# ndmarco/BayesFMMM

Measured on AMD Instinct MI355X. Metric: Gibbs iterations/sec (whole node) at n_funct=4096, K=3, P=30, higher is better.
Workload: dtype f64; 1 GPU; BFMMM_warm_start sweep, n_funct=4096, n_i=100, K=3, P=30, M=6, fp64, one independent chain per GPU (1 chain(s): a chain does not shard, replicas only); chains=1, chains_per_gpu=1

## Files before the change

### bayesfmmm_amd/_lib.py

```python
import ctypes as C
import os

_HERE = os.path.dirname(os.path.abspath(__file__))
LIB_PATH = os.environ.get("BFMMM_LIB_PATH", os.path.join(_HERE, "libbfmmm_hip.so"))

c_double_p = C.POINTER(C.c_double)
c_int64_p = C.POINTER(C.c_int64)


class BfmmmConfig(C.Structure):
    _fields_ = [("model", C.c_int32), ("n_funct", C.c_int32), ("K", C.c_int32), ("n_eigen", C.c_int32),
                ("basis_degree", C.c_int32), ("n_internal_knots", C.c_int32), ("P", C.c_int32),
                ("tot_mcmc_iters", C.c_int32), ("c", C.c_double * 8), ("b", C.c_double), ("nu_1", C.c_double),
                ("alpha1l", C.c_double), ("alpha2l", C.c_double), ("beta1l", C.c_double), ("beta2l", C.c_double),
                ("a_Z_PM", C.c_double), ("a_pi_PM", C.c_double), ("var_alpha3", C.c_double),
                ("var_epsilon1", C.c_double), ("var_epsilon2", C.c_double), ("alpha_nu", C.c_double),
                ("beta_nu", C.c_double), ("alpha_eta", C.c_double), ("beta_eta", C.c_double),
                ("alpha_0", C.c_double), ("beta_0", C.c_double)]


SYMBOLS = {
    "bfmmm_config_defaults": (None, [C.POINTER(BfmmmConfig)]),
    "bfmmm_create": (C.c_int, [C.POINTER(BfmmmConfig), C.c_int, c_double_p, c_double_p, c_int64_p, c_double_p,
                               c_double_p, C.POINTER(C.c_void_p)]),
    "bfmmm_destroy": (None, [C.c_void_p]),
    "bfmmm_create_batch": (C.c_int, [C.POINTER(BfmmmConfig), C.c_int, c_double_p, c_double_p, c_int64_p, c_double_p,
                                     c_double_p, C.c_int, C.POINTER(C.c_void_p)]),
    "bfmmm_create_from_basis_batch": (C.c_int, [C.POINTER(BfmmmConfig), C.c_int, c_double_p, c_double_p, c_int64_p, C.c_int,
                                                C.c_int, c_double_p, C.c_int, C.c_int, C.POINTER(C.c_void_p)]),
    "bfmmm_select_chain": (C.c_int, [C.c_void_p, C.c_int]),
    "bfmmm_n_chains": (C.c_int, [C.c_void_p]),
    "bfmmm_set_chain_id_stride": (C.c_int, [C.c_void_p, C.c_uint32]),
    "bfmmm_gather_best": (C.c_int, [C.POINTER(C.c_void_p), C.c_int, c_double_p, C.POINTER(C.c_int32), C.POINTER(C.c_int)]),
    "bfmmm_set_covariates": (C.c_int, [C.c_void_p, c_double_p, C.c_int, C.c_int]),
    "bfmmm_get_basis": (C.c_int, [C.c_void_p, c_double_p, C.c_int64]),
    "bfmmm_set_state": (C.c_int, [C.c_void_p, C.c_char_p, c_double_p, C.c_int64]),
    "bfmmm_get_state": (C.c_int, [C.c_void_p, C.c_char_p, c_double_p, C.c_int64]),
    "bfmmm_init_state": (C.c_int, [C.c_void_p, C.c_int, C.c_uint64, C.c_uint32]),
    "bfmmm_run": (C.c_int, [C.c_void_p, C.c_uint32, C.c_int, C.c_int, C.c_uint64, C.c_uint32, C.c_int, C.c_double]),
    "bfmmm_prepare_run": (C.c_int, [C.c_void_p, C.c_uint32, C.c_int, C.c_int, C.c_uint64, C.c_uint32, C.c_int]),
    "bfmmm_set_slot_base": (C.c_int, [C.c_void_p, C.c_int]),
    "bfmmm_create_from_basis": (C.c_int, [C.POINTER(BfmmmConfig), C.c_int, c_double_p, c_double_p, c_int64_p, C.c_int, C.c_int,
                                          c_double_p, C.c_int, C.POINTER(C.c_void_p)]),
    "bfmmm_tempered_transition": (C.c_int, [C.c_void_p, C.c_uint32, C.c_int, C.c_int, C.c_double, C.c_uint64, C.c_uint32,
                                            c_double_p, C.POINTER(C.c_int)]),
    "bfmmm_get_chain": (C.c_int, [C.c_void_p, C.c_char_p, C.c_int, c_double_p, C.c_int64]),
    "bfmmm_chain_diagnostics": (C.c_int, [C.c_void_p, C.c_char_p, C.c_int, C.c_int, C.c_int64, c_double_p, c_double_p, c_double_p,
                                          c_double_p, c_double_p, c_double_p, c_double_p, C.c_int64]),
    "bfmmm_debug_get": (C.c_int, [C.c_void_p, C.c_char_p, c_double_p, C.c_int64, c_int64_p]),
    "bfmmm_set_profile": (C.c_int, [C.c_void_p, C.c_int]),
    "bfmmm_get_timing": (C.c_int, [C.c_void_p, C.c_char_p, C.POINTER(C.c_double), c_int64_p]),
    "bfmmm_set_exact_instances": (None, [C.c_int]),
    "bfmmm_last_error": (C.c_char_p, []),
}

_LIB = None


def load():
    global _LIB
    if _LIB is None:
        if not os.path.exists(LIB_PATH):
            raise RuntimeError(
                f"{LIB_PATH} is missing: build it with `python -c 'import __graft_entry__ as g; g.build()'` "
                "(hipcc --offload-arch=gfx950). bayesfmmm_amd has no CPU fallback.")
        lib = C.CDLL(LIB_PATH)
        for name, (res, args) in SYMBOLS.items():
            fn = getattr(lib, name)
            fn.restype = res
            fn.argtypes = args
        _LIB = lib
    return _LIB


class BfmmmError(RuntimeError):
    pass


def check(rc):
    if rc != 0:
        raise BfmmmError(load().bfmmm_last_error().decode())
```

### bayesfmmm_amd/csrc/bfmmm_capi.hip

```cpp
#include "../../include/bfmmm.h"
#include "model.hpp"
#include "rng.hpp"

#include <algorithm>
#include <cmath>
#include <cstdio>
#include <cstring>
#include <map>
#include <chrono>
#include <mutex>
#include <string>
#include <tuple>
#include <vector>

namespace bfmmm {
int launch_stats_functional(int degree, int n, int P, int LREC, const int64_t* off, const double* t, const double* y,
                            const double* knots, int n_knots, double* rec, int* ni, double* B_dense, int* err,
                            hipStream_t st);
void launch_stats_multivariate(int n, int P, int LREC, const double* Y, double* rec, int* ni, hipStream_t st);
void launch_stats_totals(int n, int LREC, int yy_off, const double* rec, const int* ni, double* out_yy,
                         long long* out_counts, hipStream_t st);
int launch_curve(const Ctx& c, int which, int do_update, hipStream_t st);
int curve_blocks(int n, int P);
void prepare_curve_kernels();
// ... 921 lines not shown
  c.seed = seed; c.chain = chain; c.mask = mask;
  Plan plan = make_plan(mask, MD);
  if (c.d.D > 0) { plan.z = true; plan.chi = true; plan.use_rss_part = 1; }
  c.defer_loglik = (c.d.D == 0) ? 1 : 0;
  c.ll_use_part = plan.use_rss_part;
  h->last_md = MD;
  int nsub = 1;
  if (!h->profile && h->nch >= 4) nsub = 2;
  if (const char* env_split = h->profile ? nullptr : getenv("BFMMM_BATCH_SPLIT"))
    nsub = std::max(1, std::min({atoi(env_split), (int)bfmmm_handle::MAX_SUB, h->nch / 2}));
  Sub subs[bfmmm_handle::MAX_SUB];
  h->sub_st[0] = h->st;
  for (int q = 0, q0 = 0; q < nsub; ++q) {
    const int cnt = h->nch / nsub + (q < h->nch % nsub ? 1 : 0);
    if (pg_route(h, c.d, plan.pg, cnt, h->profile ? bfmmm_handle::MAX_SUB : q, subs[q].r)) return 1;
    if (!h->sub_st[q]) HIPCHK(hipStreamCreateWithFlags(&h->sub_st[q], hipStreamNonBlocking));
    if (!h->sub_ev[q]) HIPCHK(hipEventCreateWithFlags(&h->sub_ev[q], hipEventDisableTiming));
    subs[q].c = chain_ctx(c, (unsigned)q0);
    subs[q].c.nch = cnt;
    subs[q].st = h->sub_st[q];
    q0 += cnt;
  }
  c.defer_hyper = (c.defer_loglik && plan.pg && plan.chi && h->nch == 1 && !subs[0].r.packed && subs[0].r.NKS >= 2) ? 1 : 0;
  subs[0].c.defer_hyper = c.defer_hyper;
  if (!prepare_only) {
    ensure_sweep_tables(h, c, mask);
    hipLaunchKernelGGL(k_run_begin, dim3(h->nch), dim3(64), 0, h->st, h->c, (uint32_t)first_iter, (uint32_t)h->slot_base, tt_step, beta,
                       h->state_dirty ? 1 : 0);
    h->state_dirty = false;
    for (int f = 0; f < FAM_COUNT; ++f) { h->fam_ms[f] = 0; h->fam_launches[f] = 0; }
  }
  if (h->profile) {
    if (prepare_only) return 0;
    HIPCHK(hipEventRecord(h->ev0, h->st));
    if (run_profiled(h, c, plan, subs[0].r, n_iters, tt_step)) return 1;
    return finish_run(h, c, plan, mask, first_iter, n_iters, false);
  }
  const bool fuse = plan.z && plan.z_update && plan.chi && c.d.D == 0 && n_iters >= 2 && tt_step == 0;
  const bool defer = !fuse && plan.z && plan.z_update && plan.factor && (mask & U_Z) && c.d.D == 0 && c.d.K <= 4 && c.d.BW <= 5 &&
                     n_iters >= 2 && tt_step == 0;
  const bool bodies = fuse || defer;
  const int body_kind = fuse ? GK_FUSED : GK_DEFERRED;
  const int nrep = bodies ? n_iters - 1 : n_iters;
  const bool whole = bodies && nsub == 1 && n_iters <= WHOLE_MAX && c.defer_loglik && h->status_dev != nullptr;
  std::vector<std::pair<int, int>> segs;
  const int kind = bodies ? body_kind : GK_FULL;
  if (whole) {
    segs.push_back({GK_WHOLE, n_iters});
  } else {
    for (int q = 0; q < nrep / GRAPH_UNROLL; ++q) segs.push_back({kind, GRAPH_UNROLL});
    if (nrep % GRAPH_UNROLL) segs.push_back({kind, nrep % GRAPH_UNROLL});
    if (bodies) segs.push_back({GK_CLOSING, 1});
  }
  const bfmmm_handle::GraphKey key{mask, MD, seed, chain, nsub, bfmmm::g_exact_instances ? 1 : 0};
  if (n_iters > 0 && !(h->g_valid && h->g_key == key)) { drop_graphs(h); h->g_key = key; h->g_valid = true; }
  std::vector<FreshGraph> fresh;
  std::vector<hipGraphExec_t> seq[bfmmm_handle::MAX_SUB];
  for (int s = 0; s < nsub; ++s)
    for (const auto& sg : segs) {
      hipGraphExec_t g = nullptr;
      if (cached_graph(h, s, sg.first, sg.second, subs[s].st, fresh, [&]() { queue_graph(h, c, subs[s], plan, sg.first, sg.second, body_kind); }, &g))
        return 1;
      seq[s].push_back(g);
    }
  if (prepare_only) return dry_launch(h, c, mask, subs, nsub, fresh, first_iter, tt_step, beta);
  HIPCHK(hipEventRecord(h->ev0, h->st));
  if (nsub > 1) HIPCHK(hipEventRecord(h->evA, h->st));
  for (int q = 1; q < nsub; ++q) HIPCHK(hipStreamWaitEvent(subs[q].st, h->evA, 0));
  for (int s = 0; s < nsub && n_iters > 0; ++s) {
    if (bodies && !whole) launch_curve(subs[s].c, 0, plan.z_update, subs[s].st);
    for (hipGraphExec_t g : seq[s]) HIPCHK(hipGraphLaunch(g, subs[s].st));
  }
  for (int q = 1; q < nsub; ++q) { HIPCHK(hipEventRecord(h->sub_ev[q], subs[q].st)); HIPCHK(hipStreamWaitEvent(h->st, h->sub_ev[q], 0)); }
  return finish_run(h, c, plan, mask, first_iter, n_iters, whole);
}

extern "C" int bfmmm_set_slot_base(bfmmm_handle* h, int base) {
  if (!h || base < 0) return fail("bfmmm_set_slot_base: bad arguments");
  h->slot_base = base;
  return 0;
}

extern "C" int bfmmm_run(bfmmm_handle* h, uint32_t mask, int first_iter, int n_iters, uint64_t seed, uint32_t chain,
                         int phi_chi_zero, double beta) {
  return run_impl(h, mask, first_iter, n_iters, seed, chain, phi_chi_zero, beta, 0);
}

extern "C" int bfmmm_prepare_run(bfmmm_handle* h, uint32_t mask, int first_iter, int n_iters, uint64_t seed, uint32_t chain,
                                 int phi_chi_zero) {
  return run_impl(h, mask, first_iter, n_iters, seed, chain, phi_chi_zero, 1.0, 0, true);
}

extern "C" int bfmmm_tempered_transition(bfmmm_handle* h, uint32_t mask, int iter, int N_t, double beta_N_t,
                                         uint64_t seed, uint32_t chain, double* logA_out, int* accepted_out) {
  if (!h) return fail("bfmmm_tempered_transition: null handle");
  if (N_t < 1 || iter < h->slot_base || iter - h->slot_base >= h->T) return fail("bfmmm_tempered_transition: bad arguments");
  if (h->nch != 1) return fail("bfmmm_tempered_transition: a tempered transition accepts or rejects one chain: not available on a chain batch");
  HIPCHK(hipSetDevice(h->device));
  const Ctx& c = h->c;
  const Dims& d = c.d;
  const size_t n_th = (size_t)d.K * (d.M + 1) * d.P, n_chi = (size_t)d.n * d.M, n_Z = (size_t)d.n * d.K,
               n_dl = (size_t)d.K * d.M, n_A = (size_t)d.K * 2, n_g = (size_t)d.K * d.P * d.M;
  const size_t Dc = (size_t)d.D;
  const size_t n_tx = (size_t)d.K * (d.M + 1) * Dc * d.P, n_te = (size_t)d.K * Dc, n_gx = (size_t)d.K * d.P * Dc * d.M,
               n_dx = (size_t)d.K * d.M * Dc, n_ax = (size_t)d.K * 2 * Dc;
  if (!h->tt_save) { if (dalloc(h, &h->tt_save, n_th + n_chi + n_Z + n_dl + n_A + n_g + n_tx + n_te + n_gx + n_dx + n_ax + 8)) return 1; }
  double* sv = h->tt_save;
// ... 151 lines not shown
  HIPCHK(hipMalloc(&d_ws, per_row * (size_t)chunk));
  double* d_x = d_ws;
  double* d_out = d_x + (size_t)chunk * C * S;
  double* d_tier = d_out + 7 * (size_t)chunk;
  std::vector<double> hb(7 * (size_t)chunk);
  double* const outs[7] = {rhat, ess_bulk, ess_tail, ess_mean, mcse_mean, mean, sd};
  std::string err;
  for (int64_t p0 = 0; p0 < len && err.empty(); p0 += chunk) {
    const int rows = (int)std::min<int64_t>(chunk, len - p0);
    err = diag_gather(a->p, cb, ss, ps, first_slot, S, C, (int)p0, rows, d_x, h->st);
    if (err.empty()) err = diag_launch(d_x, rows, C, S, d_out, rows, d_tier, rows, h->st);
    if (err.empty() && copy_sync(h, hb.data(), d_out, sizeof(double) * 7 * (size_t)rows, hipMemcpyDeviceToHost) != hipSuccess)
      err = "kernel or copy back failed";
    if (err.empty())
      for (int q = 0; q < 7; ++q) std::copy(hb.begin() + (size_t)q * rows, hb.begin() + (size_t)(q + 1) * rows, outs[q] + p0);
  }
  (void)hipStreamSynchronize(h->st);
  (void)hipFree(d_ws);
  if (!err.empty()) { (void)hipGetLastError(); return fail("bfmmm_chain_diagnostics(" + s + "): " + err); }
  return 0;
}

extern "C" int bfmmm_debug_get(bfmmm_handle* h, const char* name, double* out, int64_t capacity, int64_t* count) {
  if (!h || !name || !out || !count) return fail("bfmmm_debug_get: null argument");
  HIPCHK(hipSetDevice(h->device));
  const Ctx c = selc(h);
  Dims d = c.d;
  if (h->last_md > 0) set_md(d, h->last_md);
  const std::string s(name);
  HIPCHK(hipStreamSynchronize(h->st));
  if (s == "dims") {
    const double v[] = {(double)d.n, (double)d.K, (double)d.P, (double)d.M, (double)d.BW, (double)d.LG, (double)d.LREC,
                        (double)d.MD, (double)d.A, (double)d.R, (double)d.NT, (double)d.n_obs_total, (double)d.half_sum, c.YY};
    const int64_t cnt = sizeof v / sizeof v[0];
    if (capacity < cnt) return fail("bfmmm_debug_get: buffer too small");
    memcpy(out, v, sizeof v);
    *count = cnt;
    return 0;
  }
  struct Arr { const char* nm; const double* p; int64_t len; };
  const Arr arrs[] = {{"rec", c.rec, (int64_t)d.n * d.LREC}, {"H", c.H, (int64_t)d.R * d.LG}, {"tvec", c.tvec, (int64_t)d.A * d.P},
                      {"Cmat", c.Cmat, (int64_t)d.A * d.P * d.P},
                      {"theta", c.theta, (int64_t)d.K * (d.M + 1) * d.P}};
  for (const Arr& a : arrs)
    if (s == a.nm) {
      if (capacity < a.len) return fail("bfmmm_debug_get(" + s + "): buffer too small");
      HIPCHK(copy_sync(h, out, a.p, sizeof(double) * (size_t)a.len, hipMemcpyDeviceToHost));
      *count = a.len;
      return 0;
    }
  return fail("bfmmm_debug_get: unknown name '" + s + "'");
}

namespace bfmmm { int g_exact_instances = 1; }
extern "C" void bfmmm_set_exact_instances(int enable) { bfmmm::g_exact_instances = enable ? 1 : 0; }

extern "C" int bfmmm_set_profile(bfmmm_handle* h, int enable) {
  if (!h) return fail("bfmmm_set_profile: null handle");
  h->profile = enable ? 1 : 0;
  return 0;
}

extern "C" int bfmmm_get_timing(bfmmm_handle* h, const char* name, double* ms, int64_t* launches) {
  if (!h || !name || !ms || !launches) return fail("bfmmm_get_timing: null argument");
  for (int f = 0; f < FAM_COUNT; ++f)
    if (!strcmp(name, kFamNames[f])) { *ms = h->fam_ms[f]; *launches = h->fam_launches[f]; return 0; }
  return fail("bfmmm_get_timing: unknown name");
}

#include <rccl/rccl.h>

#define NCCLCHK(x)                                                                                   \
  do {                                                                                              \
    ncclResult_t r_ = (x);                                                                          \
    if (r_ != ncclSuccess) {                                                                        \
      char buf_[512];                                                                               \
      snprintf(buf_, sizeof buf_, "RCCL error %s at %s:%d (%s)", ncclGetErrorString(r_), __FILE__, __LINE__, #x); \
      return fail(buf_);                                                                            \
    }                                                                                               \
  } while (0)

struct GatherGuard {
  std::vector<ncclComm_t> comms;
  std::vector<int> devs;
  std::vector<double*> bufs;
  ~GatherGuard() {
    for (ncclComm_t cm : comms) if (cm) (void)ncclCommDestroy(cm);
    for (size_t i = 0; i < bufs.size(); ++i)
      if (bufs[i]) { (void)hipSetDevice(devs[i / 2]); (void)hipFree(bufs[i]); }
  }
};

extern "C" int bfmmm_gather_best(bfmmm_handle* const* handles, int n_handles, const double* scores, const int32_t* chain_ids,
                                 int* winner_out) {
  if (!handles || !scores || !chain_ids || n_handles < 1) return fail("bfmmm_gather_best: bad arguments");
  const int G = n_handles;
  std::vector<int> devs(G);
  for (int g = 0; g < G; ++g) {
    if (!handles[g]) return fail("bfmmm_gather_best: null handle");
    devs[g] = handles[g]->device;
    if (handles[g]->c.chain_bytes != handles[0]->c.chain_bytes || handles[g]->c.chain_bytes_cov != handles[0]->c.chain_bytes_cov)
      return fail("bfmmm_gather_best: the handles were not created with the same configuration");
    for (int g2 = 0; g2 < g; ++g2)
      if (devs[g2] == devs[g]) return fail("bfmmm_gather_best: one handle per device");
  }
  GatherGuard gg;
  gg.devs = devs;
  gg.comms.assign(G, nullptr);
// ... 53 lines not shown
```

### bayesfmmm_amd/csrc/kernels_sweep.hip

```cpp
#include "model.hpp"
#include "rng.hpp"
#include "scalar_jobs.hpp"
#include "factor_core.hpp"
#include "z_proposal.hpp"

#include <algorithm>
#include <cstdlib>
#include <type_traits>

namespace bfmmm {



#ifdef BFMMM_TIMELINE
void fetch_fct(unsigned long long* out) { (void)hipMemcpyFromSymbol(out, HIP_SYMBOL(g_fct), sizeof(unsigned long long) * 8); }
#endif

__device__ inline void lds_barrier() { asm volatile("s_waitcnt lgkmcnt(0)\n\ts_barrier" ::: "memory"); }

#ifdef BFMMM_TIMELINE
__device__ unsigned long long g_wgtrace[3 * 1024];
void fetch_wgtrace(unsigned long long* out) { (void)hipMemcpyFromSymbol(out, HIP_SYMBOL(g_wgtrace), sizeof(unsigned long long) * 3 * 1024); }
#endif

constexpr int PG_THREADS = 512;
__host__ __device__ inline int h2_index(int P, int p, int k) { return (((k >> 1) * P + p) << 1) + (k & 1); }

template <bool BATCH, bool GROUPS>
__global__ __launch_bounds__(PG_THREADS) void k_pair_gram(Ctx c0, int KS, int nks, int do_pg, int G) {
  const int nch = BATCH ? c0.nch : 1;
  TIMELINE(c0, 1);
#ifdef BFMMM_TIMELINE
  const int wgid = blockIdx.x + gridDim.x * blockIdx.y;
  if (threadIdx.x == 0 && wgid < 1024) {
    unsigned id, hw;
    asm volatile("s_getreg_b32 %0, hwreg(HW_REG_XCC_ID)" : "=s"(id));
    asm volatile("s_getreg_b32 %0, hwreg(HW_REG_HW_ID)" : "=s"(hw));
    g_wgtrace[3 * wgid] = wall_clock64();
    g_wgtrace[3 * wgid + 1] = ((unsigned long long)(id & 0xf) << 32) | hw;
  }
  struct EndTrace { int w; __device__ ~EndTrace() { if (threadIdx.x == 0 && w < 1024) g_wgtrace[3 * w + 2] = wall_clock64(); } } et_{wgid};
#endif
  extern __shared__ __attribute__((aligned(16))) double smem[];
  const Dims& d = c0.d;
  const int n = d.n, K = d.K, MD = d.MD;
  const int ks = blockIdx.y, ct = blockIdx.x;
  if (ct == d.CTG + 1) {
    if (ks < nch && threadIdx.x < 256) {
      const Ctx c = chain_ctx(c0, (unsigned)ks);
      job_pi_alpha(c);
      TSTAMP(c, 46);
    } else if (ks >= nch && ks < 2 * nch && threadIdx.x < 256) {
      const Ctx c = chain_ctx(c0, (unsigned)(ks - nch));
      if (c.dyn->hyper_pending) {
        job_hyper(c, false);
        __syncthreads();
        if (threadIdx.x == 0) c.dyn->hyper_pending = 0u;
      }
    }
    return;
  }
  if (ks >= nks) return;
  if (!do_pg) return;
  const bool single = ct == d.CTG;
  const int ncol = single ? d.CTS * 16 : 16;
  const int col0 = single ? d.LG : ct * 16;
  const int colend = single ? d.LG + d.P : d.LG;
  const int i0 = ks * KS;
  const int RS = K + MD + 1, ONE = K;
  const int NP = d.NZZ + d.NCC, RP = NP + 1;
  const int KSP = KS + 2;
  const int KQ4 = KS >> 2;
  auto pos = [&](int il) { return (il & 3) * KQ4 + (il >> 2); };
  const int GG = GROUPS ? G : 1;
  const int TB = RS + (single ? 0 : RP);
  double* sB = smem;
  double* sW = sB + (size_t)ncol * KSP;
  double* sP = sW + (size_t)RS * KSP;
  const int tid = threadIdx.x;
  constexpr int UW = 12, UB = 6;
  const int ncw = K + MD - 1;
  const int nB = KS * ncol;
  auto loadW = [&](const double* Zq, const double* chiq, int il0, int cb, double (&v)[UW]) {
    const int i = min(i0 + il0 + tid, n - 1);
#pragma unroll
    for (int u = 0; u < UW; ++u) {
      const int col = min(cb + u, ncw - 1);
      v[u] = (col < K) ? Zq[i + (size_t)n * col] : chiq[i + (size_t)n * (col - K)];
    }
  };
  auto storeW = [&](int il0, int cb, const double (&v)[UW]) {
    const int il = il0 + tid;
    if (il >= KS) return;
    const bool live = i0 + il < n;
#pragma unroll
    for (int u = 0; u < UW; ++u) {
      const int col = cb + u;
      if (col < ncw) sW[((col < K) ? col : col + 1) * KSP + pos(il)] = live ? v[u] : 0.0;
    }
    if (cb == 0) { sW[ONE * KSP + il] = 1.0; sW[(K + MD) * KSP + il] = 0.0; }
  };
  auto loadB = [&](const double* stilq, int base, double (&v)[UB]) {
#pragma unroll
    for (int u = 0; u < UB; ++u) {
      const int q = min(base + tid + PG_THREADS * u, nB - 1);
      const int il = q / ncol, cc = q - il * ncol;
      const int i = min(i0 + il, n - 1), col = min(col0 + cc, d.LREC - 1);
      v[u] = (d.D > 0) ? stilq[(size_t)i * d.P + min(cc, d.P - 1)] : c0.rec[(size_t)i * d.LREC + col];
    }
  };
  auto storeB = [&](int base, const double (&v)[UB]) {
#pragma unroll
    for (int u = 0; u < UB; ++u) {
      const int q = base + tid + PG_THREADS * u;
      if (q < nB) {
        const int il = q / ncol, cc = q - il * ncol;
        sB[cc * KSP + pos(il)] = (i0 + il < n && col0 + cc < colend) ? v[u] : 0.0;
// ... 1546 lines not shown
    if (c.d.mv)
      ll = -(double)c.d.n * ((c.d.P / 2) * log(2 * 3.14159265358979323846 * s2)) - (1 / (s2 * 2)) * rss;
    else
      ll = -(double)c.d.n_obs_total * (0.91893853320467274178 + log(sqrt(s2))) - rss / (2.0 * s2);
    dyn->rss = rss;
    dyn->loglik = ll;
    if (c.mask & U_LOGLIK) c.c_loglik[dyn->slot] = ll;
    dyn->iter += 1;
    dyn->slot = (r_stored > 0) ? ((dyn->iter - dyn->slot_base) % (uint32_t)r_stored) : dyn->iter - dyn->slot_base;
  }
}

__global__ __launch_bounds__(256) void k_loglik_flush(Ctx c0, uint32_t* status_out) {
  const Ctx c = chain_view(c0);
  __shared__ double red[256];
  if (blockIdx.x == 1) {
    if (c.dyn->hyper_pending) {
      job_hyper(c, false);
      __syncthreads();
      if (threadIdx.x == 0) c.dyn->hyper_pending = 0u;
    }
    return;
  }
  if (c.dyn->ll_pending) deferred_loglik(c, red);
  if (status_out && threadIdx.x == 0) {
    __hip_atomic_store(&status_out[blockIdx.z], c.dyn->status, __ATOMIC_RELEASE, __HIP_MEMORY_SCOPE_SYSTEM);
  }
}

__global__ void k_fill_slots(double* chain, const double* cur, size_t len, int s0, int s1, size_t chain_bytes) {
  chain = ptr_shift(chain, blockIdx.z * chain_bytes);
  cur = ptr_shift(cur, blockIdx.z * chain_bytes);
  const size_t total = len * (size_t)(s1 - s0);
  for (size_t e = blockIdx.x * (size_t)blockDim.x + threadIdx.x; e < total; e += (size_t)gridDim.x * blockDim.x)
    chain[(size_t)s0 * len + e] = cur[e % len];
}

static size_t pair_gram_lds_bytes(const Dims& d, int KS, int G) {
  const int RS = d.K + d.MD + 1, RP = d.NZZ + d.NCC + 1;
  const size_t tables = (size_t)(KS + 2) * std::max(16 + G * (RS + RP), d.CTS * 16 + G * RS) + 128;
  return std::max(tables, (size_t)std::max(PI_ALPHA_LDS_DOUBLES, HYPER_LDS_DOUBLES)) * sizeof(double);
}
size_t pair_gram_lds_bytes(const Dims& d, int KS) { return pair_gram_lds_bytes(d, KS, 1); }

void launch_pair_gram(const Ctx& c, int do_pg, int NKS, int KS, hipStream_t st) {
  const Dims& d = c.d;
  const int ncw = d.K + d.MD - 1;
  int G = 1;
  if (c.nch > 1 && d.D == 0 && d.RT < 8)
    while (G < c.nch && pair_gram_lds_bytes(d, KS, G + 1) <= 144 * 1024 && (size_t)(G + 1) * ncw * KS <= 12 * 512) ++G;
  const size_t lds = pair_gram_lds_bytes(d, KS, G);
  if (c.nch > 1 && G > 1) hipLaunchKernelGGL((k_pair_gram<true, true>), dim3(d.CTG + 2, do_pg ? std::max(NKS, c.nch) : c.nch, 1), dim3(PG_THREADS), lds, st, c, KS, NKS, do_pg, G);
  else if (c.nch > 1) hipLaunchKernelGGL((k_pair_gram<true, false>), dim3(d.CTG + 2, do_pg ? std::max(NKS, c.nch) : c.nch, 1), dim3(PG_THREADS), lds, st, c, KS, NKS, do_pg, 1);
  else hipLaunchKernelGGL((k_pair_gram<false, false>), dim3(d.CTG + 2, do_pg ? NKS : 1, 1), dim3(PG_THREADS), lds, st, c, KS, NKS, do_pg, 1);
}

size_t pgp_lds_bytes(const PgPack& g) {
  const size_t lg = 2 * (16 * (size_t)PGP_RB + (size_t)g.NQG * 16 * g.SLS), ls = 2 * (16 * (size_t)PGP_RB + (size_t)g.NQS * 16 * g.SLS);
  return std::max(lg, ls) * sizeof(double);
}
bool pgp_geometry(const Dims& d, int nch, int KS, int NKS, PgPack& g) {
  if (d.mv || d.D > 0 || d.K > 4 || d.MD - 1 > 8 || d.P > 32 || (d.LREC & 1) || (KS & 15)) return false;
  g.KS = KS; g.NKS = NKS;
  g.NP2 = (d.LG + 31) / 32;
  g.TG = (nch * d.R + 15) / 16; g.TS = (nch * d.A + 15) / 16;
  g.WPG = PGP_WPG;
  g.NRG = (g.TG + PGP_WPG - 1) / PGP_WPG; g.NCG = (g.NP2 + 1) / 2; g.NWG_S = (g.TS + PGP_WPG - 1) / PGP_WPG;
  g.SLG = (d.NZZ + d.NCC + 1 + 1) & ~1; g.SLS = (d.K + d.MD + 1 + 1) & ~1;
  g.NQG = std::min(nch, (PGP_WPG * 16 + d.R - 2) / d.R + 1); g.NQS = std::min(nch, (PGP_WPG * 16 + d.A - 2) / d.A + 1);
  g.NTP = g.TG * 2 * g.NP2 + g.TS * 2;
  const int NV = d.K + d.MD - 1;
  if (std::max(g.NQG, g.NQS) * NV * 16 > PGP_NWV * 64 * PGP_WPG) return false;
  return pgp_lds_bytes(g) <= 64 * 1024;
}
size_t pgp_pack_doubles(const PgPack& g) { return (size_t)g.NKS * g.NTP * 256; }

void launch_pair_gram_pack(const Ctx& c, const PgPack& g, double* pack, hipStream_t st) {
  const dim3 grid(g.NRG * g.NCG + g.NWG_S, g.NKS, 1);
  hipLaunchKernelGGL(k_pair_gram_pack<PGP_WPG>, grid, dim3(64 * PGP_WPG), pgp_lds_bytes(g), st, c, g, pack);
  const int nblk_red = (g.NTP * 256 * 4 + 255) / 256;
  hipLaunchKernelGGL(k_pg_reduce_pack, dim3(nblk_red), dim3(256), 0, st, c, g, pack);
}

void launch_pg_reduce(const Ctx& c, int NKS, hipStream_t st) {
  const int nthreads = c.d.NT * 256 * 4;
  hipLaunchKernelGGL(k_pg_reduce, dim3((nthreads + 255) / 256, 1, c.nch), dim3(256), 0, st, c, NKS);
}

template <int PP>
static void launch_factor_pp(const Ctx& c, int grid, size_t lds, hipStream_t st) {
  switch (c.d.BW) {
    case 0: hipLaunchKernelGGL((k_factor<PP, 0>), dim3(c.nch * grid), dim3(256), lds, st, c); break;
    case 1: hipLaunchKernelGGL((k_factor<PP, 1>), dim3(c.nch * grid), dim3(256), lds, st, c); break;
    case 2: hipLaunchKernelGGL((k_factor<PP, 2>), dim3(c.nch * grid), dim3(256), lds, st, c); break;
    case 3: hipLaunchKernelGGL((k_factor<PP, 3>), dim3(c.nch * grid), dim3(256), lds, st, c); break;
    case 4: hipLaunchKernelGGL((k_factor<PP, 4>), dim3(c.nch * grid), dim3(256), lds, st, c); break;
    case 5: hipLaunchKernelGGL((k_factor<PP, 5>), dim3(c.nch * grid), dim3(256), lds, st, c); break;
    case BWMID: hipLaunchKernelGGL((k_factor<PP, BWMID>), dim3(c.nch * grid), dim3(256), lds, st, c); break;
    default: hipLaunchKernelGGL((k_factor<PP, BWWIDE>), dim3(c.nch * grid), dim3(256), lds, st, c); break;
  }
}

void launch_factor(const Ctx& c, hipStream_t st) {
  const int PP = (c.d.P <= 32) ? 32 : 64;
  const int W = 2 * c.d.BW + 2, PS = c.d.P + 2 * c.d.BW + 1;
  const bool diag = c.d.BW == 0 && c.d.BWP == 0;
  const size_t lds = ((diag ? 0 : 2 * (size_t)PP * PP) + (size_t)c.d.A * PS + (size_t)c.d.A * c.d.P + PP + (size_t)c.d.P * W + 16 + 4 * PP + 2) * sizeof(double);
// ... 87 lines not shown
```

### bayesfmmm_amd/csrc/model.hpp

```cpp
#pragma once
#include <hip/hip_runtime.h>
#include <stdint.h>

namespace bfmmm {

constexpr int KMAX = 8;
constexpr int PMAX = 64;
constexpr int BWMAX = 5;
constexpr int BWWIDE = 31;
constexpr int BWMID = 15;

enum : uint32_t {
  U_Z = 1u << 0, U_PI = 1u << 1, U_ALPHA3 = 1u << 2, U_PHI = 1u << 3, U_DELTA = 1u << 4, U_A = 1u << 5,
  U_GAMMA = 1u << 6, U_NU = 1u << 7, U_TAU = 1u << 8, U_SIGMA = 1u << 9, U_CHI = 1u << 10,
  U_ETA = 1u << 11, U_TAU_ETA = 1u << 12, U_XI = 1u << 13, U_DELTA_XI = 1u << 14, U_A_XI = 1u << 15,
  U_GAMMA_XI = 1u << 16, U_LOGLIK = 1u << 17
};

struct Hyper {
  double c[KMAX];
  double b, nu_1;
  double alpha1l, alpha2l, beta1l, beta2l;
  double a_Z_PM, a_pi_PM, var_alpha3, var_epsilon1, var_epsilon2;
  double alpha_nu, beta_nu, alpha_eta, beta_eta, alpha_0, beta_0;
// ... 147 lines not shown
  int covariance_adj;
  int A2;
  int NB2, NBS;
  int NPG, NPAIR;
  double *c_eta, *c_xi, *c_tau_eta, *c_gamma_xi, *c_delta_xi, *c_A_xi;
  double YY;
  size_t chain_bytes, chain_bytes_cov;
  uint32_t chain_id_stride;
  int nch;
  double *c_nu, *c_chi, *c_Z, *c_pi, *c_alpha3, *c_delta, *c_A, *c_sigma, *c_tau, *c_gamma, *c_Phi, *c_loglik;
  int nblk_curve;
};

struct PgPack {
  int KS, NKS;
  int TG, TS;
  int NRG, NCG, NWG_S;
  int SLG, SLS;
  int NQG, NQS;
  int WPG;
  int NTP;
  int NP2;
};

#define BFMMM_CHAIN_PTRS(X_)                                                                                         \
  X_(dyn) X_(Z) X_(chi) X_(theta) X_(delta) X_(Aa) X_(gamma) X_(logz_part) X_(rss_part) X_(pg_part) X_(H) X_(H2)       \
  X_(tvec) X_(rvec) X_(hq) X_(Lz) X_(gstd) X_(zprep) X_(chi_norm) X_(piprep) X_(Cmat)                        \
  X_(c_nu) X_(c_chi) X_(c_Z) X_(c_pi) X_(c_alpha3) X_(c_delta) X_(c_A) X_(c_sigma) X_(c_tau) X_(c_gamma) X_(c_Phi) X_(c_loglik)
#define BFMMM_CHAIN_PTRS_COV(X_)                                                                                     \
  X_(thetaX) X_(tau_eta) X_(gamma_xi) X_(delta_xi) X_(A_xi) X_(stil) X_(yyp_part) X_(cfull) X_(gfull) X_(w2_part)      \
  X_(H2aa) X_(gstd2) X_(Wdir) X_(C2) X_(Lz2) X_(step_part) X_(thetaN) X_(delta_cur)                                   \
  X_(c_eta) X_(c_xi) X_(c_tau_eta) X_(c_gamma_xi) X_(c_delta_xi) X_(c_A_xi)

template <typename T>
__host__ __device__ inline T* ptr_shift(T* p, size_t bytes) { return (T*)((char*)p + bytes); }

__host__ __device__ inline Ctx chain_ctx(const Ctx& c0, unsigned q) {
  Ctx c = c0;
  const size_t o1 = (size_t)q * c0.chain_bytes, o2 = (size_t)q * c0.chain_bytes_cov;
#define X_(f) c.f = ptr_shift(c0.f, o1);
  BFMMM_CHAIN_PTRS(X_)
#undef X_
#define X_(f) c.f = ptr_shift(c0.f, o2);
  BFMMM_CHAIN_PTRS_COV(X_)
#undef X_
  c.chain = c0.chain + q * c0.chain_id_stride;
  return c;
}
#ifdef __HIPCC__
__device__ inline Ctx chain_view(const Ctx& c0) { return chain_ctx(c0, blockIdx.z); }
#endif

extern int g_exact_instances;

__host__ __device__ inline int tri_index(int n, int a, int b) {
  return a * n - (a * (a - 1)) / 2 + (b - a);
}

#ifdef BFMMM_TIMELINE
struct Timeline {
  unsigned long long* s; int k;
  __device__ Timeline(const Ctx& c, int k_) : s(c.dyn->stamps), k(k_) {
    if (blockIdx.x == 0 && blockIdx.y == 0 && threadIdx.x == 0) s[2 * k] = wall_clock64();
    if (threadIdx.x == 0) atomicMax(&s[16 + k], (unsigned long long)wall_clock64());
  }
  __device__ ~Timeline() { if (threadIdx.x == 0) atomicMax(&s[2 * k + 1], (unsigned long long)wall_clock64()); }
};
#define TIMELINE(c, k) Timeline tl_((c), (k))
#define TSTAMP(c, i) do { if (threadIdx.x == 0) atomicMax(&(c).dyn->stamps[i], (unsigned long long)wall_clock64()); } while (0)
#define TSTAMP0(c, i) do { if (threadIdx.x == 0 && blockIdx.x == 0 && blockIdx.y == 0) (c).dyn->stamps[i] = wall_clock64(); } while (0)
#else
#define TIMELINE(c, k) do { } while (0)
#define TSTAMP(c, i) do { } while (0)
#define TSTAMP0(c, i) do { } while (0)
#endif

template <int CTRL>
__device__ inline double dpp_add(double v) {
  const int lo = __builtin_amdgcn_update_dpp(0, __double2loint(v), CTRL, 0xf, 0xf, true);
  const int hi = __builtin_amdgcn_update_dpp(0, __double2hiint(v), CTRL, 0xf, 0xf, true);
  return v + __hiloint2double(hi, lo);
}
__device__ inline double row16_sum(double v) {
  v = dpp_add<0xB1>(v);
  v = dpp_add<0x4E>(v);
  v = dpp_add<0x141>(v);
  v = dpp_add<0x140>(v);
  return v;
}

template <int LPC>
__device__ inline double group_sum(double v) {
  v = row16_sum(v);
  v += __shfl_xor(v, 16, 64);
  if (LPC == 64) v += __shfl_xor(v, 32, 64);
  return v;
}

template <int UN>
__device__ inline void copy_to_lds(double* dst, const double* __restrict__ src, int count, int tid, int nthreads) {
  for (int base = 0; base < count; base += nthreads * UN) {
    double v[UN];
#pragma unroll
    for (int u = 0; u < UN; ++u) v[u] = src[min(base + tid + nthreads * u, count - 1)];
#pragma unroll
    for (int u = 0; u < UN; ++u) {
// ... 15 lines not shown
```

### include/bfmmm.h

```cpp
#ifndef BFMMM_H
#define BFMMM_H

#include <stdint.h>

#ifdef __cplusplus
extern "C" {
#endif

typedef struct bfmmm_handle bfmmm_handle;

enum { BFMMM_MODEL_FUNCTIONAL = 0, BFMMM_MODEL_MULTIVARIATE = 1 };

enum {
  BFMMM_U_Z = 1 << 0, BFMMM_U_PI = 1 << 1, BFMMM_U_ALPHA3 = 1 << 2, BFMMM_U_PHI = 1 << 3,
  BFMMM_U_DELTA = 1 << 4, BFMMM_U_A = 1 << 5, BFMMM_U_GAMMA = 1 << 6, BFMMM_U_NU = 1 << 7,
  BFMMM_U_TAU = 1 << 8, BFMMM_U_SIGMA = 1 << 9, BFMMM_U_CHI = 1 << 10,
  BFMMM_U_ETA = 1 << 11, BFMMM_U_TAU_ETA = 1 << 12, BFMMM_U_XI = 1 << 13, BFMMM_U_DELTA_XI = 1 << 14,
  BFMMM_U_A_XI = 1 << 15, BFMMM_U_GAMMA_XI = 1 << 16, BFMMM_U_LOGLIK = 1 << 17
};
#define BFMMM_SWEEP_NU_Z  (BFMMM_U_Z | BFMMM_U_PI | BFMMM_U_ALPHA3 | BFMMM_U_NU | BFMMM_U_TAU | BFMMM_U_SIGMA | BFMMM_U_LOGLIK)
#define BFMMM_SWEEP_THETA (BFMMM_U_PHI | BFMMM_U_DELTA | BFMMM_U_A | BFMMM_U_GAMMA | BFMMM_U_TAU | BFMMM_U_SIGMA | BFMMM_U_CHI | BFMMM_U_LOGLIK)
#define BFMMM_SWEEP_WARM  (BFMMM_SWEEP_NU_Z | BFMMM_SWEEP_THETA)
#define BFMMM_COV_MEAN (BFMMM_U_ETA | BFMMM_U_TAU_ETA)
#define BFMMM_COV_XI   (BFMMM_U_XI | BFMMM_U_DELTA_XI | BFMMM_U_A_XI | BFMMM_U_GAMMA_XI)
// ... 16 lines not shown

void bfmmm_config_defaults(bfmmm_config* cfg);

int bfmmm_create(const bfmmm_config* cfg, int device, const double* y, const double* t, const int64_t* offsets,
                 const double* internal_knots, const double* boundary_knots, bfmmm_handle** out);

int bfmmm_create_from_basis(const bfmmm_config* cfg, int device, const double* y, const double* B, const int64_t* offsets,
                            int P, int band, const double* Pmat, int pen_band, bfmmm_handle** out);
void bfmmm_destroy(bfmmm_handle* h);

int bfmmm_create_batch(const bfmmm_config* cfg, int device, const double* y, const double* t, const int64_t* offsets,
                       const double* internal_knots, const double* boundary_knots, int n_chains, bfmmm_handle** out);
int bfmmm_create_from_basis_batch(const bfmmm_config* cfg, int device, const double* y, const double* B, const int64_t* offsets,
                                  int P, int band, const double* Pmat, int pen_band, int n_chains, bfmmm_handle** out);
int bfmmm_select_chain(bfmmm_handle* h, int q);
int bfmmm_n_chains(const bfmmm_handle* h);
int bfmmm_set_chain_id_stride(bfmmm_handle* h, uint32_t stride);

int bfmmm_gather_best(bfmmm_handle* const* handles, int n_handles, const double* scores, const int32_t* chain_ids, int* winner);

int bfmmm_set_covariates(bfmmm_handle* h, const double* X, int D, int covariance_adj);

int bfmmm_get_basis(bfmmm_handle* h, double* out, int64_t capacity);

int bfmmm_set_state(bfmmm_handle* h, const char* name, const double* values, int64_t count);
int bfmmm_get_state(bfmmm_handle* h, const char* name, double* out, int64_t capacity);

int bfmmm_init_state(bfmmm_handle* h, int stage, uint64_t seed, uint32_t chain);

int bfmmm_run(bfmmm_handle* h, uint32_t mask, int first_iter, int n_iters, uint64_t seed, uint32_t chain,
              int phi_chi_zero, double beta);

int bfmmm_prepare_run(bfmmm_handle* h, uint32_t mask, int first_iter, int n_iters, uint64_t seed, uint32_t chain,
                      int phi_chi_zero);

int bfmmm_set_slot_base(bfmmm_handle* h, int base);

int bfmmm_tempered_transition(bfmmm_handle* h, uint32_t mask, int iter, int N_t, double beta_N_t, uint64_t seed,
                              uint32_t chain, double* logA, int* accepted);

int bfmmm_get_chain(bfmmm_handle* h, const char* name, int n_slots, double* out, int64_t capacity);

int bfmmm_chain_diagnostics(bfmmm_handle* h, const char* name, int first_slot, int n_slots, int64_t max_workspace_bytes,
                            double* rhat, double* ess_bulk, double* ess_tail, double* ess_mean, double* mcse_mean,
                            double* mean, double* sd, int64_t capacity);

int bfmmm_debug_get(bfmmm_handle* h, const char* name, double* out, int64_t capacity, int64_t* count);

int bfmmm_set_profile(bfmmm_handle* h, int enable);
int bfmmm_get_timing(bfmmm_handle* h, const char* name, double* ms, int64_t* launches);

void bfmmm_set_exact_instances(int enable);

const char* bfmmm_last_error(void);

#ifdef __cplusplus
}
#endif
#endif
```

Before: 17660 Gibbs iterations/sec.

## Add solo-chain pair-Gram path using FP64 MFMA with double-buffered LDS tiles

```diff
diff --git a/bayesfmmm_amd/_lib.py b/bayesfmmm_amd/_lib.py
--- a/bayesfmmm_amd/_lib.py
+++ b/bayesfmmm_amd/_lib.py
@@ -51,6 +51,7 @@
     "bfmmm_set_profile": (C.c_int, [C.c_void_p, C.c_int]),
     "bfmmm_get_timing": (C.c_int, [C.c_void_p, C.c_char_p, C.POINTER(C.c_double), c_int64_p]),
     "bfmmm_set_exact_instances": (None, [C.c_int]),
+    "bfmmm_set_solo_pair_gram": (None, [C.c_int]),
     "bfmmm_last_error": (C.c_char_p, []),
 }
 
diff --git a/bayesfmmm_amd/csrc/bfmmm_capi.hip b/bayesfmmm_amd/csrc/bfmmm_capi.hip
--- a/bayesfmmm_amd/csrc/bfmmm_capi.hip
+++ b/bayesfmmm_amd/csrc/bfmmm_capi.hip
@@ -997,7 +997,7 @@
     if (nrep % GRAPH_UNROLL) segs.push_back({kind, nrep % GRAPH_UNROLL});
     if (bodies) segs.push_back({GK_CLOSING, 1});
   }
-  const bfmmm_handle::GraphKey key{mask, MD, seed, chain, nsub, bfmmm::g_exact_instances ? 1 : 0};
+  const bfmmm_handle::GraphKey key{mask, MD, seed, chain, nsub, (bfmmm::g_exact_instances ? 1 : 0) | (bfmmm::g_solo_pair_gram ? 2 : 0)};
   if (n_iters > 0 && !(h->g_valid && h->g_key == key)) { drop_graphs(h); h->g_key = key; h->g_valid = true; }
   std::vector<FreshGraph> fresh;
   std::vector<hipGraphExec_t> seq[bfmmm_handle::MAX_SUB];
@@ -1255,8 +1255,9 @@
   return fail("bfmmm_debug_get: unknown name '" + s + "'");
 }
 
-namespace bfmmm { int g_exact_instances = 1; }
+namespace bfmmm { int g_exact_instances = 1; int g_solo_pair_gram = 1; }
 extern "C" void bfmmm_set_exact_instances(int enable) { bfmmm::g_exact_instances = enable ? 1 : 0; }
+extern "C" void bfmmm_set_solo_pair_gram(int enable) { bfmmm::g_solo_pair_gram = enable ? 1 : 0; }
 
 extern "C" int bfmmm_set_profile(bfmmm_handle* h, int enable) {
   if (!h) return fail("bfmmm_set_profile: null handle");
diff --git a/bayesfmmm_amd/csrc/kernels_sweep.hip b/bayesfmmm_amd/csrc/kernels_sweep.hip
--- a/bayesfmmm_amd/csrc/kernels_sweep.hip
+++ b/bayesfmmm_amd/csrc/kernels_sweep.hip
@@ -25,6 +25,143 @@
 
 constexpr int PG_THREADS = 512;
 __host__ __device__ inline int h2_index(int P, int p, int k) { return (((k >> 1) * P + p) << 1) + (k & 1); }
+
+constexpr int PG_SOLO = 2;
+constexpr int PGS_TMAX = 4;
+constexpr int PGS_KS = 256;
+
+inline bool pg_solo_fits(const Dims& d, int KS) {
+  return !d.mv && d.D == 0 && d.K <= 4 && d.MD - 1 <= 8 && d.P <= 32 && d.LG <= 128 && KS <= PGS_KS &&
+         d.RT <= PGS_TMAX * (PG_THREADS / 64);
+}
+
+template <int NTL>
+__device__ inline void pg_solo_tiles(const double* sP, const double* sB, int KSP, int KQ, int nchunk, const int (&o1)[PGS_TMAX],
+                                     const int (&o2)[PGS_TMAX], int lr, int kq, double4_t (&acc)[PGS_TMAX]) {
+  const v2d* pa[NTL]; const v2d* pb[NTL];
+#pragma unroll
+  for (int q = 0; q < NTL; ++q) {
+    pa[q] = (const v2d*)(sP + o1[q] * KSP + kq * KQ);
+    pb[q] = (const v2d*)(sP + o2[q] * KSP + kq * KQ);
+  }
+  const v2d* pc = (const v2d*)(sB + lr * KSP + kq * KQ);
+  struct Ops { v2d a[2][NTL], b[2][NTL], c[2]; };
+  auto load = [&](Ops& o, int t) {
+#pragma unroll
+    for (int u = 0; u < 2; ++u) {
+      o.c[u] = pc[2 * t + u];
+#pragma unroll
+      for (int q = 0; q < NTL; ++q) { o.a[u][q] = pa[q][2 * t + u]; o.b[u][q] = pb[q][2 * t + u]; }
+    }
+  };
+  auto mfma = [&](const Ops& o) {
+#pragma unroll
+    for (int u = 0; u < 2; ++u)
+#pragma unroll
+      for (int q = 0; q < NTL; ++q) {
+        acc[q] = __builtin_amdgcn_mfma_f64_16x16x4f64(o.a[u][q].x * o.b[u][q].x, o.c[u].x, acc[q], 0, 0, 0);
+        acc[q] = __builtin_amdgcn_mfma_f64_16x16x4f64(o.a[u][q].y * o.b[u][q].y, o.c[u].y, acc[q], 0, 0, 0);
+      }
+  };
+  Ops s0, s1;
+  load(s0, 0);
+  for (int t = 0; t < nchunk; t += 2) {
+    if (t + 1 < nchunk) load(s1, t + 1);
+    __builtin_amdgcn_sched_barrier(0);
+    mfma(s0);
+    __builtin_amdgcn_sched_barrier(0);
+    if (t + 2 < nchunk) load(s0, t + 2);
+    __builtin_amdgcn_sched_barrier(0);
+    if (t + 1 < nchunk) mfma(s1);
+    __builtin_amdgcn_sched_barrier(0);
+  }
+}
+
+__device__ inline void pg_solo_g(const Ctx& c0, int KS, int ks, int ct, double* smem) {
+  const Dims& d = c0.d;
+  const int n = d.n, K = d.K, MD = d.MD, tid = threadIdx.x;
+#ifdef BFMMM_TIMELINE
+  struct { Dyn* dyn; } c = {c0.dyn};
+#endif
+  TSTAMP0(c, 40);
+  const int i0 = ks * KS;
+  const int nlive = min(KS, n - i0);
+  const int nchunk = (nlive + 15) >> 4;
+  const int nst = nchunk * 16;
+  const int KSP = KS + 2, KQ = KS >> 2;
+  const int NZZ = d.NZZ, NP = NZZ + d.NCC;
+  double* sB = smem;
+  double* sP = sB + 16 * KSP;
+  const bool wl = tid < nlive;
+  const int iw = i0 + tid;
+  double z[4], x[8];
+#pragma unroll
+  for (int a = 0; a < 4; ++a) z[a] = (wl && a < K) ? c0.Z[iw + (size_t)n * a] : 0.0;
+#pragma unroll
+  for (int m = 0; m < 8; ++m) x[m] = (wl && m < MD - 1) ? c0.chi[iw + (size_t)n * m] : 0.0;
+  const int ccg = tid & 15, ilg = tid >> 4;
+  const bool colok = ct * 16 + ccg < d.LG;
+  const double* srcg = c0.rec + (size_t)i0 * d.LREC + min(ct * 16 + ccg, d.LREC - 1);
+  double vb[PGS_KS / 32];
+#pragma unroll
+  for (int u = 0; u < PGS_KS / 32; ++u) {
+    const int il = ilg + 32 * u;
+    vb[u] = (il < nlive && colok) ? srcg[(size_t)il * d.LREC] : 0.0;
+  }
+  TSTAMP0(c, 47);
+  if (tid < nst) {
+    double* dst = sP + (tid & 3) * KQ + (tid >> 2);
+    int e = 0;
+#pragma unroll
+    for (int a = 0; a < 4; ++a)
+#pragma unroll
+      for (int b = a; b < 4; ++b)
+        if (b < K) { dst[e * KSP] = z[a] * z[b]; ++e; }
+    const double xt[9] = {1.0, x[0], x[1], x[2], x[3], x[4], x[5], x[6], x[7]};
+#pragma unroll
+    for (int a = 0; a < 9; ++a)
+#pragma unroll
+      for (int b = a; b < 9; ++b)
+        if (b < MD) { dst[e * KSP] = xt[a] * xt[b]; ++e; }
+    dst[NP * KSP] = 0.0;
+  }
+#pragma unroll
+  for (int u = 0; u < PGS_KS / 32; ++u) {
+    const int il = ilg + 32 * u;
+    if (il < nst) sB[ccg * KSP + (il & 3) * KQ + (il >> 2)] = vb[u];
+  }
+  TSTAMP0(c, 41);
+  lds_barrier();
+  TSTAMP0(c, 42);
+  constexpr int NW = PG_THREADS / 64;
+  const int wave = tid >> 6, lane = tid & 63, lr = lane & 15, kq = lane >> 4;
+  const int ntl = __builtin_amdgcn_readfirstlane(max(0, min(PGS_TMAX, (d.RT - wave + NW - 1) / NW)));
+  int o1[PGS_TMAX], o2[PGS_TMAX];
+#pragma unroll
+  for (int q = 0; q < PGS_TMAX; ++q) {
+    const int row = (wave + NW * q) * 16 + lr;
+    o1[q] = o2[q] = NP;
+    if (q < ntl && row < d.R) { const int zz = row / d.NCC; o1[q] = zz; o2[q] = NZZ + (row - zz * d.NCC); }
+  }
+  double4_t acc[PGS_TMAX];
+#pragma unroll
+  for (int q = 0; q < PGS_TMAX; ++q) acc[q] = double4_t{0.0, 0.0, 0.0, 0.0};
+  switch (ntl) {
+    case 1: pg_solo_tiles<1>(sP, sB, KSP, KQ, nchunk, o1, o2, lr, kq, acc); break;
+    case 2: pg_solo_tiles<2>(sP, sB, KSP, KQ, nchunk, o1, o2, lr, kq, acc); break;
+    case 3: pg_solo_tiles<3>(sP, sB, KSP, KQ, nchunk, o1, o2, lr, kq, acc); break;
+    case 4: pg_solo_tiles<4>(sP, sB, KSP, KQ, nchunk, o1, o2, lr, kq, acc); break;
+    default: break;
+  }
+#pragma unroll
+  for (int q = 0; q < PGS_TMAX; ++q)
+    if (q < ntl) {
+      double* out = c0.pg_part + ((size_t)ks * d.NT + (size_t)(wave + NW * q) * d.CTG + ct) * 256 + lane;
+      __builtin_nontemporal_store(acc[q][0], out); __builtin_nontemporal_store(acc[q][1], out + 64);
+      __builtin_nontemporal_store(acc[q][2], out + 128); __builtin_nontemporal_store(acc[q][3], out + 192);
+    }
+  TSTAMP0(c, 44);
+}
 
 template <bool BATCH, bool GROUPS>
 __global__ __launch_bounds__(PG_THREADS) void k_pair_gram(Ctx c0, int KS, int nks, int do_pg, int G) {
@@ -63,6 +200,9 @@
   if (ks >= nks) return;
   if (!do_pg) return;
   const bool single = ct == d.CTG;
+  if constexpr (!BATCH) {
+    if (do_pg == PG_SOLO && !single) { pg_solo_g(c0, KS, ks, ct, smem); return; }
+  }
   const int ncol = single ? d.CTS * 16 : 16;
   const int col0 = single ? d.LG : ct * 16;
   const int colend = single ? d.LG + d.P : d.LG;
@@ -1715,7 +1855,10 @@
   const size_t lds = pair_gram_lds_bytes(d, KS, G);
   if (c.nch > 1 && G > 1) hipLaunchKernelGGL((k_pair_gram<true, true>), dim3(d.CTG + 2, do_pg ? std::max(NKS, c.nch) : c.nch, 1), dim3(PG_THREADS), lds, st, c, KS, NKS, do_pg, G);
   else if (c.nch > 1) hipLaunchKernelGGL((k_pair_gram<true, false>), dim3(d.CTG + 2, do_pg ? std::max(NKS, c.nch) : c.nch, 1), dim3(PG_THREADS), lds, st, c, KS, NKS, do_pg, 1);
-  else hipLaunchKernelGGL((k_pair_gram<false, false>), dim3(d.CTG + 2, do_pg ? NKS : 1, 1), dim3(PG_THREADS), lds, st, c, KS, NKS, do_pg, 1);
+  else {
+    const int pg = (do_pg && g_solo_pair_gram && pg_solo_fits(d, KS)) ? PG_SOLO : do_pg;
+    hipLaunchKernelGGL((k_pair_gram<false, false>), dim3(d.CTG + 2, do_pg ? NKS : 1, 1), dim3(PG_THREADS), lds, st, c, KS, NKS, pg, 1);
+  }
 }
 
 size_t pgp_lds_bytes(const PgPack& g) {
diff --git a/bayesfmmm_amd/csrc/model.hpp b/bayesfmmm_amd/csrc/model.hpp
--- a/bayesfmmm_amd/csrc/model.hpp
+++ b/bayesfmmm_amd/csrc/model.hpp
@@ -223,6 +223,7 @@
 #endif
 
 extern int g_exact_instances;
+extern int g_solo_pair_gram;
 
 __host__ __device__ inline int tri_index(int n, int a, int b) {
   return a * n - (a * (a - 1)) / 2 + (b - a);
diff --git a/include/bfmmm.h b/include/bfmmm.h
--- a/include/bfmmm.h
+++ b/include/bfmmm.h
@@ -92,6 +92,8 @@
 
 void bfmmm_set_exact_instances(int enable);
 
+void bfmmm_set_solo_pair_gram(int enable);
+
 const char* bfmmm_last_error(void);
 
 #ifdef __cplusplus
```

After: 18430 Gibbs iterations/sec, median of 6. 1.04x the previous value.
